# TimoStoff/event_utils

Measured on AMD Instinct MI355X. Metric: Mevents/s (voxel 5-bin 640x480), higher is better.
Workload: dtype f32

## Files before the change

### event_utils_amd/csrc/evk_part.h

```cpp
#pragma once
#include "evk_tiles.h"

namespace evk {

#define EVK_WAIT_VM0() __builtin_amdgcn_s_waitcnt(0x0F70)

struct TileGridG {
    int tw, th, pitch;
    int tiles_x, tiles_y;
    int dom_w, dom_h;
    float ix, iy;
    uint32_t mx, mp;
};
__host__ __device__ inline uint32_t magic_div(uint32_t d) { return (uint32_t)((((uint64_t)1 << 32) + d - 1) / d); }
__device__ __forceinline__ uint32_t div_magic(uint32_t x, uint32_t m) { return __umulhi(x, m); }
#define EVK_GRIDG_MAX_CELLS 1024

__device__ __forceinline__ int tile_of(int u, float inv) { return (int)(((float)u + 0.5f) * inv); }

static inline int make_grid_g(TileGridG &g, int dom_h, int dom_w, int tw, int th) {
    if (dom_h <= 0 || dom_w <= 0 || dom_h > 65535 || dom_w > 65535 || tw < 4 || th < 4 || tw > 256 || th > 256 ||
        (tw | 1) * th > EVK_GRIDG_MAX_CELLS)
        return EVK_EINVAL;
    g.tw = tw, g.th = th, g.pitch = tw | 1;
    g.dom_w = dom_w, g.dom_h = dom_h;
    g.tiles_x = (dom_w + tw - 1) / tw;
    g.tiles_y = (dom_h + th - 1) / th;
    g.ix = 1.0f / (float)tw, g.iy = 1.0f / (float)th;
    g.mx = magic_div((uint32_t)tw), g.mp = magic_div((uint32_t)(tw * th));
    return EVK_OK;
}

template <bool WRAP = true>
__device__ __forceinline__ int nearest_key_cell_int(int xi, int yi, bool finite, const TileGridG &g, uint32_t &cell) {
    if constexpr (WRAP) {
        xi += xi < 0 ? g.dom_w : 0;
        yi += yi < 0 ? g.dom_h : 0;
    }
    const bool ok = finite & ((uint32_t)xi < (uint32_t)g.dom_w) & ((uint32_t)yi < (uint32_t)g.dom_h);
    const int ux = ok ? xi : 0, uy = ok ? yi : 0;
    const int tx = tile_of(ux, g.ix), ty = tile_of(uy, g.iy);
    cell = (uint32_t)(__mul24(uy - __mul24(ty, g.th), g.pitch) + (ux - __mul24(tx, g.tw)));
    return ok ? __mul24(ty, g.tiles_x) + tx : -1;
}
__device__ __forceinline__ int nearest_key_cell(float x, float y, const TileGridG &g, uint32_t &cell) {
    return nearest_key_cell_int((int)x, (int)y, (x == x) & (y == y), g, cell);
}

struct TimeNorm {
    float t_first, dt, bm1;
};
__host__ __device__ inline TimeNorm make_time_norm(float t_first, float t_last, float bm1) {
    return TimeNorm{t_first, t_last - t_first, bm1};
}
__device__ __forceinline__ float time_norm(float t, const TimeNorm &k) { return (t - k.t_first) / k.dt * k.bm1; }

typedef uint32_t evk_u32x4 __attribute__((ext_vector_type(4)));
struct __attribute__((packed, aligned(4))) evk_quad4 {
    evk_u32x4 v;
};
template <bool NT>
__device__ __forceinline__ uint4 load_col16(const float *col, int64_t ev0, uint32_t gl) {
    const evk_quad4 *q = reinterpret_cast<const evk_quad4 *>(col + ev0) + gl;
    evk_u32x4 v;
#pragma clang diagnostic push
#pragma clang diagnostic ignored "-Waddress-of-packed-member"
    if constexpr (NT) v = __builtin_nontemporal_load(&q->v);
    else v = q->v;
#pragma clang diagnostic pop
    return make_uint4(v.x, v.y, v.z, v.w);
}
struct SrcF32 {
    static constexpr int G = 4, XYW = 8, TPW = 8;
    const float *x, *y, *t, *p;
    template <bool NT = false>
    __device__ __forceinline__ void load_xy(int64_t ev0, uint32_t gl, uint32_t *r) const {
        const uint4 a = load_col16<NT>(x, ev0, gl), b = load_col16<NT>(y, ev0, gl);
        r[0] = a.x, r[1] = a.y, r[2] = a.z, r[3] = a.w, r[4] = b.x, r[5] = b.y, r[6] = b.z, r[7] = b.w;
    }
    template <bool NT = false>
    __device__ __forceinline__ void load_tp(int64_t ev0, uint32_t gl, uint32_t *r) const {
        const uint4 a = load_col16<NT>(t, ev0, gl), b = load_col16<NT>(p, ev0, gl);
        r[0] = a.x, r[1] = a.y, r[2] = a.z, r[3] = a.w, r[4] = b.x, r[5] = b.y, r[6] = b.z, r[7] = b.w;
    }
    __device__ __forceinline__ int key_of(const uint32_t *r, int e, const TileGridG &g, uint32_t &cell) const {
        return nearest_key_cell(__uint_as_float(r[e]), __uint_as_float(r[4 + e]), g, cell);
    }
    __device__ __forceinline__ float t_of(const uint32_t *r, int e) const { return __uint_as_float(r[e]); }
    __device__ __forceinline__ float p_of(const uint32_t *r, int e) const { return __uint_as_float(r[4 + e]); }
    __device__ __forceinline__ float t1(int64_t i) const { return t[i]; }
};

template <bool T64>
struct SrcNative {
    static constexpr int G = 4, XYW = 4, TPW = T64 ? 9 : 5;
    const int16_t *x, *y;
    const void *t;
    const uint8_t *p;
    double t_offset;
    int xy_stride, p_kind;
    template <bool NT = false>
    __device__ __forceinline__ void load_xy(int64_t ev0, uint32_t gl, uint32_t *r) const {
        if (xy_stride == 2) {
            const uint4 w = reinterpret_cast<const uint4 *>(x + 2 * ev0)[gl];
            r[0] = w.x, r[1] = w.y, r[2] = w.z, r[3] = w.w;
        } else {
            const uint2 a = reinterpret_cast<const uint2 *>(x + ev0)[gl], b = reinterpret_cast<const uint2 *>(y + ev0)[gl];
            r[0] = a.x, r[1] = a.y, r[2] = b.x, r[3] = b.y;
        }
    }
    template <bool NT = false>
    __device__ __forceinline__ void load_tp(int64_t ev0, uint32_t gl, uint32_t *r) const {
        if constexpr (T64) {
            const uint4 a = reinterpret_cast<const uint4 *>(static_cast<const double *>(t) + ev0)[2 * gl];
            const uint4 b = reinterpret_cast<const uint4 *>(static_cast<const double *>(t) + ev0)[2 * gl + 1];
            r[0] = a.x, r[1] = a.y, r[2] = a.z, r[3] = a.w, r[4] = b.x, r[5] = b.y, r[6] = b.z, r[7] = b.w;
        } else {
            const uint4 a = reinterpret_cast<const uint4 *>(static_cast<const float *>(t) + ev0)[gl];
            r[0] = a.x, r[1] = a.y, r[2] = a.z, r[3] = a.w;
        }
        r[TPW - 1] = reinterpret_cast<const uint32_t *>(p + ev0)[gl];
    }
    __device__ __forceinline__ int key_of(const uint32_t *r, int e, const TileGridG &g, uint32_t &cell) const {
        const uint32_t wx = xy_stride == 2 ? r[e] << 16 : (e & 1 ? r[e >> 1] : r[e >> 1] << 16);
        const uint32_t wy = xy_stride == 2 ? r[e] : (e & 1 ? r[2 + (e >> 1)] : r[2 + (e >> 1)] << 16);
        return nearest_key_cell_int((int32_t)wx >> 16, (int32_t)wy >> 16, true, g, cell);
    }
    __device__ __forceinline__ float t_of(const uint32_t *r, int e) const {
        if constexpr (T64) {
            const double d = __hiloint2double((int)r[2 * e + 1], (int)r[2 * e]);
            return (float)(d - t_offset);
        } else {
            return (float)((double)__uint_as_float(r[e]) - t_offset);
        }
    }
    __device__ __forceinline__ float p_of(const uint32_t *r, int e) const {
        const uint32_t b = (r[TPW - 1] >> (8 * e)) & 0xffu;
        return p_kind == EVK_P_U8_PM1 ? (float)(2 * (int)b - 1) : (p_kind == EVK_P_I8 ? (float)(int8_t)b : (float)b);
    }
    __device__ __forceinline__ float t1(int64_t i) const {
        return (float)((T64 ? static_cast<const double *>(t)[i] : (double)static_cast<const float *>(t)[i]) - t_offset);
    }
};

}
```

### event_utils_amd/csrc/evk_part2.h

```cpp
#pragma once
#include <cstdio>
#include <cstring>
#include <mutex>
#include <type_traits>

#include "evk_part.h"

namespace evk {

#define V2_HDR 16
#define V2_MAX_TILES 2048
#define V2_TOTALS V2_HDR
#define V2_LIVE_PROGRESS (V2_HDR + V2_MAX_TILES)
#define V2_LIVE_STATUS (V2_LIVE_PROGRESS + 256)
#define V2_PART (V2_LIVE_STATUS + V2_MAX_TILES)
#define V2_COUNTER(T) (V2_PART + (T) + 1)
#define V2_ITEM(T) (V2_PART + 2 * (T) + 1)
#define V2_LB 10
#define EVK_VOXEL2_COUNT (1 << 20)
#define EVK_VOXEL2_COUNT2 (1 << 21)
#define V2_LOCAL_MASK ((1u << V2_LB) - 1u)
#define V2_WIDE (1u << V2_LB)
#define V2_P_MASK (~((2u << V2_LB) - 1u))
__device__ __forceinline__ void lds_barrier() { asm volatile("s_waitcnt lgkmcnt(0)\n\ts_barrier" ::: "memory"); }

template <int THREADS>
__device__ __forceinline__ uint32_t block_excl_scan(uint32_t mine, uint32_t *tmp, uint32_t &total) {
    constexpr int NW = THREADS / 64;
    const int lane = threadIdx.x & 63, wave = threadIdx.x >> 6;
    uint32_t incl = mine;
#pragma unroll
    for (int off = 1; off < 64; off <<= 1) {
        const uint32_t v = __shfl_up(incl, off, 64);
        if (lane >= off) incl += v;
    }
    if (lane == 63) tmp[wave] = incl;
    lds_barrier();
    if (wave == 0) {
        const uint32_t w = lane < NW ? tmp[lane] : 0u;
        uint32_t wi = w;
#pragma unroll
        for (int off = 1; off < NW; off <<= 1) {
            const uint32_t v = __shfl_up(wi, off, 64);
            if (lane >= off) wi += v;
        }
        if (lane < NW) tmp[32 + lane] = wi - w;
        if (lane == NW - 1) tmp[64] = wi;
    }
    lds_barrier();
    total = tmp[64];
    return tmp[32 + wave] + incl - mine;
}

__host__ __device__ static inline int64_t v2_staging_stride(int64_t cells) { return (cells + 31) & ~(int64_t)31; }

struct Part2 {
    int S;
    int per_block;
    int nsc;
    int nt_pad;
    int nblk;
};

#define V2_FMT_IMGN 1
#define V2_FMT_IMGB 12
#define V2_FMT_IMGT 13
#define V2_FMT_IMGX 14
#define V2_FMT_IMGD 15
#define V2_FMT_VOX8W 9
#define V2_DELTA_SHIFT 12
#define V2_DELTA_LIMIT (1u << 20)
#define V2_CODE_SHIFT 10
__host__ __device__ constexpr int v2_fmt_lds_bytes(int rec) { return rec == V2_FMT_IMGN ? 8 : ((rec == V2_FMT_VOX8W || rec == V2_FMT_IMGT || rec == V2_FMT_IMGX || rec == V2_FMT_IMGD) ? 12 : rec); }
template <int THREADS, int EPT, int REC, typename C, bool LIVE = false>
__global__ void __launch_bounds__(THREADS, 4) k_part_sorted(const C c, int64_t n, TileGridG g, int ntiles, Part2 q, float t_first,
                                                            float t_last, float bm1, int t_from_events,
                                                            void *__restrict__ rec_, void *__restrict__ side_,
                                                            uint32_t *__restrict__ bases,
                                                            uint32_t *__restrict__ table, uint32_t *__restrict__ index,
                                                            uint32_t cap, uint32_t part, uint32_t *oob, uint32_t *host_report,
                                                            uint32_t seq, uint32_t *live_progress = nullptr,
                                                            uint32_t live_epoch = 0) {
    static_assert(!LIVE || REC == 8, "the live consumer reads 8-byte records written through");
    static_assert(REC == 8 || REC == 4 || REC == V2_FMT_IMGN || REC == V2_FMT_IMGB || REC == V2_FMT_IMGT || REC == V2_FMT_IMGX || REC == V2_FMT_IMGD || REC == V2_FMT_VOX8W, "record format");
    constexpr bool R8 = REC == 8 || REC == V2_FMT_VOX8W;
    constexpr bool IMGBT = REC == V2_FMT_IMGB || REC == V2_FMT_IMGT || REC == V2_FMT_IMGX || REC == V2_FMT_IMGD;
    constexpr bool STAGE_W = REC == V2_FMT_VOX8W || REC == V2_FMT_IMGN || IMGBT;
    constexpr bool VOX = R8 || REC == 4;
    constexpr int LB = v2_fmt_lds_bytes(REC);
    uint2 *const rec = static_cast<uint2 *>(rec_);
    float *const pw = static_cast<float *>(side_);
    uint2 *const wide2 = static_cast<uint2 *>(side_);
    constexpr int G = C::G, NG = EPT / G;
    static_assert(EPT % G == 0, "events per thread");
    constexpr int PER_MAX = (V2_MAX_TILES + THREADS - 1) / THREADS;
    extern __shared__ __attribute__((aligned(16))) unsigned char smem[];
    uint2 *sorted = reinterpret_cast<uint2 *>(smem);
    uint32_t *hist = reinterpret_cast<uint32_t *>(smem + (size_t)THREADS * EPT * LB + 16);
    uint32_t *cur = hist + ((ntiles + 4) & ~3);
    uint32_t *tot = cur + ((ntiles + 4) & ~3);
    uint32_t *tmp = tot + ((ntiles + 4) & ~3);
    uint32_t *trow_l = tmp + 72 + 4;
    uint32_t *sorted4 = reinterpret_cast<uint32_t *>(smem);
    uint32_t *sortedp = reinterpret_cast<uint32_t *>(smem + (size_t)THREADS * EPT * (REC == V2_FMT_IMGN ? 4 : 8));
    __shared__ int is_last;
    const int tid = threadIdx.x, lane = tid & 63;
    uint32_t dropped = 0, nwide = 0;
    float tb = 0.0f;
    if constexpr (VOX) {
        if (t_from_events) t_first = c.t1(0), t_last = c.t1(n - 1);
    }
    const TimeNorm tnorm = make_time_norm(t_first, t_last, bm1);
    float ts_a = 0.0f, ts_d = 1.0f;
    if constexpr (REC == V2_FMT_IMGT) c.time_constants(n, t_from_events, ts_a, ts_d);
    constexpr bool EARLY = !IMGBT;
    uint32_t early_prev = 0;
    auto early_publish = [&]() {
        EVK_HANDOVER_ACQUIRE();
        __hip_atomic_store(index + 8, 0u, __ATOMIC_RELAXED, __HIP_MEMORY_SCOPE_AGENT);
        if (host_report) {
            const uint32_t cnt = oob ? __hip_atomic_load(oob, __ATOMIC_RELAXED, __HIP_MEMORY_SCOPE_AGENT) : 0u;
            __hip_atomic_store(reinterpret_cast<unsigned long long *>(host_report),
                               (unsigned long long)seq | ((unsigned long long)cnt << 32), __ATOMIC_RELAXED, __HIP_MEMORY_SCOPE_SYSTEM);
        }
    };

    int tl_ = tid;
    auto valid_in = [&](int sc, int k) -> int {
        const int64_t lo = (int64_t)sc * q.S;
        const int64_t hi = (lo + q.S < n) ? lo + q.S : n;
        return (int)(hi - lo) - G * (tl_ + k * THREADS);
    };
    auto row_base = [&](int sc, int k) -> int64_t {
        const int64_t lo = (int64_t)sc * q.S, hi = (lo + q.S < n) ? lo + q.S : n, r = lo + (int64_t)G * k * THREADS;
        return r < hi ? r : lo;
    };
    const int sc0 = blockIdx.x * q.per_block;
    const int sc_end = (sc0 + q.per_block < q.nsc) ? sc0 + q.per_block : q.nsc;
    uint32_t xyr[NG * C::XYW], tpr[NG * C::TPW];
    float tv[EPT];
    uint32_t kl[EPT];
    float xr[EPT], yr[EPT];
    uint32_t rare = 0;
    auto load_xy = [&](int sc) {
#pragma unroll
        for (int k = 0; k < NG; ++k) c.template load_xy<true>(row_base(sc, k), valid_in(sc, k) > 0 ? (uint32_t)tl_ : 0u, xyr + C::XYW * k);
    };
    auto load_tp = [&](int sc) {
#pragma unroll
        for (int k = 0; k < NG; ++k) c.template load_tp<true>(row_base(sc, k), valid_in(sc, k) > 0 ? (uint32_t)tl_ : 0u, tpr + C::TPW * k);
        if constexpr (REC == 4) tb = c.t1((int64_t)sc * q.S);
    };
    auto fence = [&]() {
        asm volatile("" ::: "memory");
        __builtin_amdgcn_sched_barrier(0);
    };
    for (int i = tid; i < ntiles; i += THREADS) hist[i] = 0, tot[i] = 0;
    if (tid < 8) tmp[64 + tid] = 0;
    if (sc0 < sc_end) load_xy(sc0);
    EVK_WAIT_VM0();
    lds_barrier();
    uint32_t kept_prev = 0;
    int64_t lo_prev = 0;
    int sc_prev = 0;
    auto store_run = [&](const uint4 *src, uint4 *dst, const int n16) {
        if constexpr (REC != 4) {
            typedef uint32_t u4v __attribute__((ext_vector_type(4)));
            const __amdgpu_buffer_rsrc_t rs = __builtin_amdgcn_make_buffer_rsrc(
                (void *)dst, 0, (int)__builtin_amdgcn_readfirstlane(n16 * 16), 0x00020000);
            for (int i = tid; i < n16; i += THREADS) {
                const uint4 v = src[i];
                __builtin_amdgcn_raw_buffer_store_b128(u4v{v.x, v.y, v.z, v.w}, rs, i * 16, 0,  16);
            }
        } else {
            for (int i = tid; i < n16; i += THREADS) dst[i] = src[i];
        }
    };
    auto write_out = [&]() {
        const uint4 *src = reinterpret_cast<const uint4 *>(sorted);
        if constexpr (R8 || IMGBT)
            store_run(src, reinterpret_cast<uint4 *>(rec + lo_prev), (int)((kept_prev + 1) >> 1));
        else
            store_run(src, reinterpret_cast<uint4 *>(reinterpret_cast<uint32_t *>(rec_) + lo_prev), (int)((kept_prev + 3) >> 2));
        if constexpr (LIVE)
            store_run(reinterpret_cast<const uint4 *>(trow_l), reinterpret_cast<uint4 *>(table + (int64_t)sc_prev * q.nt_pad), q.nt_pad >> 2);
        if constexpr (STAGE_W) {
            if (tmp[65])
                store_run(reinterpret_cast<const uint4 *>(sortedp),
                          reinterpret_cast<uint4 *>(static_cast<uint32_t *>(side_) + lo_prev), (int)((kept_prev + 3) >> 2));
        }
    };
    for (int sc = sc0; sc < sc_end; ++sc) {
        asm volatile("" : "+v"(tl_));
        const int64_t lo = (int64_t)sc * q.S;
        if (sc > sc0) write_out();
#pragma unroll
        for (int k = 0; k < NG; ++k) {
            const int nv = valid_in(sc, k);
#pragma unroll
            for (int e = 0; e < G; ++e) {
                uint32_t cell = 0;
                int key;
                if constexpr (IMGBT) key = c.key_rel(xyr + C::XYW * k, e, g, xr[G * k + e], yr[G * k + e]);
                else key = c.key_of(xyr + C::XYW * k, e, g, cell);
                kl[G * k + e] = ((key >= 0) & (e < nv)) ? (((uint32_t)key << V2_LB) | cell) : 0xFFFFFFFFu;
                if constexpr (VOX) dropped += ((key < 0) & (e < nv)) ? 1u : 0u;
                else dropped += ((key == -1) & (e < nv)) ? 1u : 0u;
                if constexpr (IMGBT) rare |= ((key == -3) & (e < nv)) ? (1u << (G * k + e)) : 0u;
                asm volatile("" : "+v"(dropped));
                __builtin_amdgcn_sched_barrier(0);
            }
        }
#pragma unroll
        for (int s2 = 0; s2 < EPT; ++s2) asm volatile("" : "+v"(kl[s2])::"memory");
        load_tp(sc);
#pragma unroll
        for (int s2 = 0; s2 < EPT; ++s2)
            if (kl[s2] != 0xFFFFFFFFu)
                __hip_atomic_fetch_add(&hist[kl[s2] >> V2_LB], 1u, __ATOMIC_RELAXED, __HIP_MEMORY_SCOPE_WORKGROUP);
        if constexpr (EARLY) {
            if (sc == sc_end - 1 && dropped) __hip_atomic_fetch_add(&tmp[69], dropped, __ATOMIC_RELAXED, __HIP_MEMORY_SCOPE_WORKGROUP);
        }
        lds_barrier();
        if constexpr (EARLY) {
            if (sc == sc_end - 1 && tid == 0 && oob && tmp[69])
                __hip_atomic_fetch_add(oob, tmp[69], __ATOMIC_RELAXED, __HIP_MEMORY_SCOPE_AGENT);
        }
        uint32_t kept = 0;
        {
            uint32_t *trow = table + (int64_t)sc * q.nt_pad;
            constexpr int NWV = THREADS / 64;
            const int wave = tid >> 6;
            for (int base = 0; base < ntiles; base += THREADS) {
                const int i = base + tid;
                const uint32_t cnt = i < ntiles ? hist[i] : 0u;
                uint32_t incl = cnt;
#pragma unroll
                for (int off = 1; off < 64; off <<= 1) {
                    const uint32_t v = __shfl_up(incl, off, 64);
                    if (lane >= off) incl += v;
                }
                if (lane == 63) tmp[wave] = incl;
                lds_barrier();
                const uint32_t wt = lane < NWV ? tmp[lane] : 0u;
                uint32_t wi = wt;
#pragma unroll
                for (int off = 1; off < NWV; off <<= 1) {
                    const uint32_t v = __shfl_up(wi, off, 64);
                    if (lane >= off) wi += v;
                }
                const uint32_t carry = kept + __shfl(wi - wt, wave, 64);
                if (i < ntiles) {
                    const uint32_t start = carry + incl - cnt;
                    cur[i] = start;
                    hist[i] = 0;
                    tot[i] += cnt;
                    if constexpr (LIVE) trow_l[i] = start | (cnt << 16);
                    else trow[i] = start | (cnt << 16);
                }
                kept += __shfl(wi, NWV - 1, 64);
                if (base + THREADS < ntiles) lds_barrier();
            }
            if (REC == 4 && tid == 0) tmp[67] = 0;
            if (STAGE_W && tid == 0) tmp[65] = 0;
        }
        lds_barrier();
        if constexpr (VOX) {
#pragma unroll
            for (int s2 = 0; s2 < EPT; ++s2) {
                tv[s2] = time_norm(c.t_of(tpr + C::TPW * (s2 / G), s2 % G), tnorm);
                __builtin_amdgcn_sched_barrier(0);
            }
        }
        EVK_WAIT_VM0();
        fence();
        if constexpr (EARLY) {
            if (sc == sc_end - 1 && tid == 0) {
                EVK_HANDOVER_RELEASE();
                early_prev = __hip_atomic_fetch_add(index + 8, 1u, __ATOMIC_RELAXED, __HIP_MEMORY_SCOPE_AGENT);
            }
        }
        if (sc + 1 < sc_end) load_xy(sc + 1);
        fence();
        uint32_t pos_[EPT];
#pragma unroll
        for (int s2 = 0; s2 < EPT; ++s2) {
            pos_[s2] = 0;
            if (kl[s2] != 0xFFFFFFFFu) pos_[s2] = atomicAdd(&cur[kl[s2] >> V2_LB], 1u);
        }
        auto slot_of = [&](int s2) -> uint32_t { return pos_[s2]; };
        if constexpr (REC == V2_FMT_VOX8W) {
            bool any_wide = false;
#pragma unroll
            for (int s2 = 0; s2 < EPT; ++s2) {
                if (kl[s2] != 0xFFFFFFFFu) {
                    const uint32_t pos = slot_of(s2);
                    const uint32_t pbits = __float_as_uint(c.p_of(tpr + C::TPW * (s2 / G), s2 % G));
                    const bool wide = ((pbits & ~V2_P_MASK) != 0u) | ((pbits & 0x7F800000u) == 0x7F800000u);
                    nwide += ((((pbits & 0x7FFFFFFFu) == 0x3F800000u) | (pbits == 0u)) ? 0u : 0x10000u) + (wide ? 1u : 0u);
                    sorted[pos] = make_uint2(__float_as_uint(tv[s2]), (wide ? V2_WIDE : (pbits & V2_P_MASK)) | (kl[s2] & V2_LOCAL_MASK));
                    sortedp[pos] = pbits;
                    any_wide |= wide;
                }
            }
            if (any_wide) tmp[65] = 1u;
        } else if constexpr (REC == 8) {
            uint32_t wide_mask = 0;
#pragma unroll
            for (int s2 = 0; s2 < EPT; ++s2) {
                if (kl[s2] != 0xFFFFFFFFu) {
                    const uint32_t pos = slot_of(s2);
                    const uint32_t pbits = __float_as_uint(c.p_of(tpr + C::TPW * (s2 / G), s2 % G));
                    const bool wide = ((pbits & ~V2_P_MASK) != 0u) | ((pbits & 0x7F800000u) == 0x7F800000u);
                    nwide += (((pbits & 0x7FFFFFFFu) == 0x3F800000u) | (pbits == 0u)) ? 0u : 0x10000u;
                    sorted[pos] = make_uint2(__float_as_uint(tv[s2]), (wide ? V2_WIDE : (pbits & V2_P_MASK)) | (kl[s2] & V2_LOCAL_MASK));
                    if (wide) wide_mask |= 1u << s2, kl[s2] = pos;
                }
            }
            if (__any(wide_mask != 0u)) {
#pragma unroll
                for (int s2 = 0; s2 < EPT; ++s2)
                    if (wide_mask >> s2 & 1u) pw[lo + kl[s2]] = c.p_of(tpr + C::TPW * (s2 / G), s2 % G), ++nwide;
            }
        } else if constexpr (REC == V2_FMT_IMGN) {
            bool any_wide = false;
#pragma unroll
            for (int s2 = 0; s2 < EPT; ++s2) {
                if (kl[s2] != 0xFFFFFFFFu) {
                    const uint32_t pos = slot_of(s2);
                    bool wide, unit;
                    const uint32_t pay = c.payload(tpr + C::TPW * (s2 / G), s2 % G, wide, unit);
                    nwide += (unit ? 0u : 0x10000u) + (wide ? 1u : 0u);
                    sorted4[pos] = (wide ? V2_WIDE : (pay & V2_P_MASK)) | (kl[s2] & V2_LOCAL_MASK);
                    sortedp[pos] = c.w_bits(tpr + C::TPW * (s2 / G), s2 % G);
                    any_wide |= wide;
                }
            }
            if (any_wide) tmp[65] = 1u;
        } else if constexpr (REC == V2_FMT_IMGB || REC == V2_FMT_IMGX) {
            bool any_b = false;
#pragma unroll
            for (int s2 = 0; s2 < EPT; ++s2) {
                if (kl[s2] != 0xFFFFFFFFu) {
                    const uint32_t pos = slot_of(s2);
                    const uint32_t wb = c.w_bits(tpr + C::TPW * (s2 / G), s2 % G);
                    const uint32_t code = (wb & 0x7FFFFFFFu) == 0x3F800000u ? wb >> 31 : 3u - (uint32_t)(wb == 0u);
                    nwide += code == 3u ? 0x10001u : 0u;
                    sorted[pos] = make_uint2((__float_as_uint(xr[s2]) & 0x7FFFFFFFu) | (code << 31),
                                             (__float_as_uint(yr[s2]) & 0x7FFFFFFFu) | ((code >> 1) << 31));
                    sortedp[pos] = wb;
                    any_b |= code == 3u;
                }
            }
            if (any_b) tmp[65] = 1u;
            if (__any(rare != 0u)) {
#pragma unroll
                for (int s2 = 0; s2 < EPT; ++s2)
                    if (rare >> s2 & 1u) {
                        if constexpr (REC == V2_FMT_IMGX)
                            dropped += c.rare_at(row_base(sc, s2 / G) + (int64_t)G * tl_ + (s2 % G)) ? 0u : 1u;
                        else
                            dropped += c.rare(xr[s2], yr[s2], __uint_as_float(c.w_bits(tpr + C::TPW * (s2 / G), s2 % G))) ? 0u : 1u;
                    }
            }
            rare = 0;
        } else if constexpr (REC == V2_FMT_IMGD) {
            bool any_d = false;
#pragma unroll
            for (int s2 = 0; s2 < EPT; ++s2) {
                if (kl[s2] != 0xFFFFFFFFu) {
                    const uint32_t pos = slot_of(s2);
                    sorted[pos] = make_uint2(__float_as_uint(xr[s2]), __float_as_uint(yr[s2]));
                    sortedp[pos] = (uint32_t)(row_base(sc, s2 / G) + (int64_t)G * tl_ + (s2 % G));
                    any_d = true;
                }
            }
            if (any_d) tmp[65] = 1u;
            if (__any(rare != 0u)) {
#pragma unroll
                for (int s2 = 0; s2 < EPT; ++s2)
                    if (rare >> s2 & 1u) dropped += c.rare_at(row_base(sc, s2 / G) + (int64_t)G * tl_ + (s2 % G)) ? 0u : 1u;
            }
            rare = 0;
        } else if constexpr (REC == V2_FMT_IMGT) {
            bool any_t = false;
#pragma unroll
            for (int s2 = 0; s2 < EPT; ++s2) {
                if (kl[s2] != 0xFFFFFFFFu) {
                    const uint32_t pos = slot_of(s2);
                    const uint32_t cls = c.cls(tpr + C::TPW * (s2 / G), s2 % G);
                    sorted[pos] = make_uint2((__float_as_uint(xr[s2]) & 0x7FFFFFFFu) | ((cls & 1u) << 31),
                                             (__float_as_uint(yr[s2]) & 0x7FFFFFFFu) | ((cls >> 1) << 31));
                    sortedp[pos] = c.nts_bits(tpr + C::TPW * (s2 / G), s2 % G, ts_a, ts_d);
                    any_t = true;
                }
            }
            if (any_t) tmp[65] = 1u;
            if (__any(rare != 0u)) {
#pragma unroll
                for (int s2 = 0; s2 < EPT; ++s2)
                    if (rare >> s2 & 1u) dropped += c.rare_ts(xr[s2], yr[s2], tpr + C::TPW * (s2 / G), s2 % G, ts_a, ts_d) ? 0u : 1u;
            }
            rare = 0;
        } else {
            const uint32_t bbits = __float_as_uint(time_norm(tb, tnorm));
            if (tid == 0) bases[sc] = bbits;
#pragma unroll
            for (int s2 = 0; s2 < EPT; ++s2) {
                const uint32_t tbits = __float_as_uint(tv[s2]), pb = __float_as_uint(c.p_of(tpr + C::TPW * (s2 / G), s2 % G));
                const uint32_t d = tbits - bbits;
                const uint32_t code = (pb & 0x7FFFFFFFu) == 0x3F800000u ? pb >> 31 : 3u - (uint32_t)(pb == 0u);
                const bool live = kl[s2] != 0xFFFFFFFFu;
                nwide += (live & (code == 3u)) ? 0x10000u : 0u;
                const bool esc = live & ((code == 3u) | (d >= V2_DELTA_LIMIT));
                uint32_t word = (d << V2_DELTA_SHIFT) | (code << V2_CODE_SHIFT) | (kl[s2] & V2_LOCAL_MASK);
                if (__any(esc)) {
                    if (esc) {
                        const uint32_t e = atomicAdd(&tmp[67], 1u);
                        wide2[lo + e] = make_uint2(tbits, pb);
                        word = (e << V2_DELTA_SHIFT) | (3u << V2_CODE_SHIFT) | (kl[s2] & V2_LOCAL_MASK);
                        ++nwide;
                    }
                }
                if (live) sorted4[slot_of(s2)] = word;
            }
        }
        lds_barrier();
        if constexpr (EARLY) {
            if (sc == sc_end - 1 && tid == 0 && early_prev == gridDim.x - 1) early_publish();
        }
        if constexpr (LIVE) {
            if (sc > sc0 && tid == 0)
                __hip_atomic_store(live_progress + blockIdx.x, (live_epoch << 8) | (uint32_t)(sc - sc0), __ATOMIC_RELAXED,
                                   __HIP_MEMORY_SCOPE_AGENT);
        }
        EVK_WAIT_VM0();
        kept_prev = kept, lo_prev = lo, sc_prev = sc;
    }
    uint32_t *gidx = index;
    if constexpr (EARLY) {
        if (sc0 >= sc_end && tid == 0) {
            early_prev = __hip_atomic_fetch_add(index + 8, 1u, __ATOMIC_RELAXED, __HIP_MEMORY_SCOPE_AGENT);
            if (early_prev == gridDim.x - 1) early_publish();
        }
    } else {
        if (dropped && oob) atomicAdd(oob, dropped);
    }
    for (int i = tid; i < ntiles; i += THREADS)
        if (tot[i]) __hip_atomic_fetch_add(gidx + V2_TOTALS + i, tot[i], __ATOMIC_RELAXED, __HIP_MEMORY_SCOPE_AGENT);
    {
        uint32_t nw = nwide & 0xFFFFu, nu = nwide >> 16;
#pragma unroll
        for (int off = 32; off >= 1; off >>= 1) nw += __shfl_xor(nw, off, 64), nu += __shfl_xor(nu, off, 64);
        if (lane == 0) {
            if (nw) __hip_atomic_fetch_add(&tmp[66], nw, __ATOMIC_RELAXED, __HIP_MEMORY_SCOPE_WORKGROUP);
            if (nu) __hip_atomic_fetch_add(&tmp[68], nu, __ATOMIC_RELAXED, __HIP_MEMORY_SCOPE_WORKGROUP);
        }
    }
    if (sc0 < sc_end) write_out();
    lds_barrier();
    if (tid == 0) {
        const uint32_t nw = tmp[66], nu = tmp[68];
        if (nw) __hip_atomic_fetch_add(gidx + 3, nw, __ATOMIC_RELAXED, __HIP_MEMORY_SCOPE_AGENT);
        if (nu) __hip_atomic_fetch_add(gidx + 5, nu, __ATOMIC_RELAXED, __HIP_MEMORY_SCOPE_AGENT);
    }
    if constexpr (VOX) {
        if (blockIdx.x == 0 && tid == 0 && n > 0) {
            __hip_atomic_store(gidx + 0, __float_as_uint(c.t1(0)), __ATOMIC_RELAXED, __HIP_MEMORY_SCOPE_AGENT);
            __hip_atomic_store(gidx + 1, __float_as_uint(c.t1(n - 1)), __ATOMIC_RELAXED, __HIP_MEMORY_SCOPE_AGENT);
        }
    }
    EVK_HANDOVER_DRAIN();
    if constexpr (LIVE) {
        if (sc0 < sc_end && tid == 0)
            __hip_atomic_store(live_progress + blockIdx.x, (live_epoch << 8) | (uint32_t)(sc_end - sc0), __ATOMIC_RELAXED,
                               __HIP_MEMORY_SCOPE_AGENT);
    }
    if (tid == 0) {
        const uint32_t prev = __hip_atomic_fetch_add(gidx + 2, 1u, __ATOMIC_RELAXED, __HIP_MEMORY_SCOPE_AGENT);
        is_last = (prev == gridDim.x - 1);
    }
    __syncthreads();
    if (!is_last) return;
    EVK_HANDOVER_ACQUIRE();
    const int per = (ntiles + THREADS - 1) / THREADS;
    const int i0 = tid * per, i1 = (i0 + per < ntiles) ? i0 + per : ntiles;
    uint32_t *part_start = index + V2_PART, *counters = index + V2_COUNTER(ntiles), *item_tile = index + V2_ITEM(ntiles);
    uint32_t tt[PER_MAX];
    uint32_t np = 0;
    uint32_t now5 = 0, prev6 = 0, cnt_oob = 0, now3 = 0, prev0 = 0;
    if (tid == 0) {
        now5 = __hip_atomic_load(gidx + 5, __ATOMIC_RELAXED, __HIP_MEMORY_SCOPE_AGENT);
        prev6 = __hip_atomic_load(gidx + 6, __ATOMIC_RELAXED, __HIP_MEMORY_SCOPE_AGENT);
        if constexpr (!VOX) {
            now3 = __hip_atomic_load(gidx + 3, __ATOMIC_RELAXED, __HIP_MEMORY_SCOPE_AGENT);
            prev0 = __hip_atomic_load(gidx + 0, __ATOMIC_RELAXED, __HIP_MEMORY_SCOPE_AGENT);
        }
        if (!EARLY && host_report && oob) cnt_oob = __hip_atomic_load(oob, __ATOMIC_RELAXED, __HIP_MEMORY_SCOPE_AGENT);
    }
#pragma unroll
    for (int k = 0; k < PER_MAX; ++k) {
        const int i = i0 + k;
        tt[k] = 0;
        if (k < per && i < i1) {
            tt[k] = __hip_atomic_load(gidx + V2_TOTALS + i, __ATOMIC_RELAXED, __HIP_MEMORY_SCOPE_AGENT);
            __hip_atomic_store(gidx + V2_TOTALS + i, 0u, __ATOMIC_RELAXED, __HIP_MEMORY_SCOPE_AGENT);
            np += tt[k] > cap ? (tt[k] + part - 1) / part : 1u;
        }
    }
    uint32_t total_parts;
    uint32_t prun = block_excl_scan<THREADS>(np, tmp, total_parts);
#pragma unroll
    for (int k = 0; k < PER_MAX; ++k) {
        const int i = i0 + k;
        if (k < per && i < i1) {
            const uint32_t parts = tt[k] > cap ? (tt[k] + part - 1) / part : 1u;
            part_start[i] = prun;
            counters[i] = 0;
            for (uint32_t jj = 0; jj < parts; ++jj) item_tile[prun + jj] = (uint32_t)i;
            prun += parts;
        }
    }
    if (tid == 0) {
        part_start[ntiles] = total_parts;
        __hip_atomic_store(gidx + 2, 0u, __ATOMIC_RELAXED, __HIP_MEMORY_SCOPE_AGENT);
        __hip_atomic_store(gidx + 7, now5 != prev6 ? 1u : 0u, __ATOMIC_RELAXED, __HIP_MEMORY_SCOPE_AGENT);
        __hip_atomic_store(gidx + 6, now5, __ATOMIC_RELAXED, __HIP_MEMORY_SCOPE_AGENT);
        if constexpr (!VOX) {
            __hip_atomic_store(gidx + 1, now3 != prev0 ? 1u : 0u, __ATOMIC_RELAXED, __HIP_MEMORY_SCOPE_AGENT);
            __hip_atomic_store(gidx + 0, now3, __ATOMIC_RELAXED, __HIP_MEMORY_SCOPE_AGENT);
        }
        if (!EARLY && host_report) {
            const uint32_t cnt = cnt_oob;
            __hip_atomic_store(reinterpret_cast<unsigned long long *>(host_report),
                               (unsigned long long)seq | ((unsigned long long)cnt << 32), __ATOMIC_RELAXED, __HIP_MEMORY_SCOPE_SYSTEM);
        }
    }
}

struct V2Config {
    int threads, ept;
};
#define V2_GEOMETRIES(X) X(1024, 8) X(1024, 12)
static const V2Config &v2_config(bool share = false, int ntiles = 0) {
    static const V2Config small{1024, 8}, large{1024, 12};
    return (share || ntiles <= 680) ? small : large;
}
#define V2_MIN_SUBCHUNK 8192
#define V2_LDS_LIMIT (160 * 1024 - 512)
static size_t v2_part_lds(int threads, int ept, int rec, int ntiles, bool live = false) {
    return (size_t)threads * ept * v2_fmt_lds_bytes(rec) + 16 + 3 * (size_t)((ntiles + 4) & ~3) * 4 + 72 * 4 + 16 +
           (live ? (size_t)((ntiles + 15) & ~15) * 4 + 16 : 0);
}

static Part2 v2_geometry(int64_t n, int ntiles, bool share = false) {
    const V2Config &c = v2_config(share, ntiles);
    const int64_t smax = (int64_t)c.threads * c.ept;
    int64_t nblk = (n + V2_MIN_SUBCHUNK - 1) / V2_MIN_SUBCHUNK;
    const int64_t maxblk = (int64_t)EVK_NUM_CU * (1024 / c.threads);
    if (nblk > maxblk) nblk = maxblk;
    if (nblk < 1) nblk = 1;
    int64_t per_block = (n + nblk * smax - 1) / (nblk * smax);
    if (per_block < 1) per_block = 1;
    int64_t S = (n + nblk * per_block - 1) / (nblk * per_block);
    S = (S + 3) & ~(int64_t)3;
    if (S < 4) S = 4;
    Part2 q;
    q.S = (int)S, q.per_block = (int)per_block, q.nblk = (int)nblk;
    q.nsc = (int)((n + S - 1) / S);
    if (q.nsc < 1) q.nsc = 1;
    q.nt_pad = (ntiles + 15) & ~15;
    return q;
}
static inline int64_t al256(int64_t b) { return (b + 255) & ~(int64_t)255; }

#define V2_SPLIT_AT 2.5
#define V2_SPLIT_PART 1.6
static int64_t v2_mean(int64_t n, int ntiles) { return n / (ntiles > 0 ? ntiles : 1); }
static int64_t v2_cap(int64_t n, int ntiles) {
    const int64_t c = (int64_t)(V2_SPLIT_AT * (double)v2_mean(n, ntiles));
    return c > 16384 ? c : 16384;
}
static int64_t v2_part(int64_t n, int ntiles) {
    const int64_t c = (int64_t)(V2_SPLIT_PART * (double)v2_mean(n, ntiles));
    return c > 8192 ? c : 8192;
}
static int v2_max_items(int64_t n, int ntiles) { return ntiles + (int)(n / v2_part(n, ntiles)) + 1; }

static int v2_rec_bytes(int64_t n, int flags) {
    if (flags & EVK_VOXEL2_REC4) return 4;
    if (flags & EVK_VOXEL2_REC8) return 8;
    return n * 16 > ((int64_t)256 << 20) ? 4 : 8;
}
struct V2Layout {
    int64_t table, bases, rec, pw, staging, total;
};
static V2Layout v2_layout(int ntiles, int64_t n, int planes, int tw, int th, bool share = false) {
    const Part2 q = v2_geometry(n, ntiles, share);
    const int64_t slots = (int64_t)q.nsc * q.S;
    V2Layout L;
    L.table = 0;
    L.bases = al256((int64_t)q.nsc * q.nt_pad * 4);
    L.rec = L.bases + al256((int64_t)q.nsc * 4);
    L.pw = L.rec + al256(slots * 8);
    L.staging = L.pw + al256(slots * 8);
    L.total = L.staging + al256((int64_t)v2_max_items(n, ntiles) * v2_staging_stride((int64_t)planes * tw * th) * 8);
    return L;
}

template <int THREADS, int EPT, int REC, typename C, bool LIVE = false>
static void launch_part(const C &c, int64_t n, const TileGridG &g, int ntiles, const Part2 &q, float t_first, float t_last,
                        float bm1, int t_from_events, void *rec, void *pw, uint32_t *bases, uint32_t *table, uint32_t *index,
                        uint32_t *oob, uint32_t *host_report, uint32_t seq, hipStream_t s, uint32_t *live_progress = nullptr,
                        uint32_t live_epoch = 0) {
    const size_t lds = v2_part_lds(THREADS, EPT, REC, ntiles, LIVE);
    static std::once_flag once[64];
    int dev = 0;
    (void)hipGetDevice(&dev);
    std::call_once(once[dev & 63], [] {
        (void)hipFuncSetAttribute((const void *)k_part_sorted<THREADS, EPT, REC, C, LIVE>, hipFuncAttributeMaxDynamicSharedMemorySize,
                                  160 * 1024 - 256);
    });
    k_part_sorted<THREADS, EPT, REC, C, LIVE><<<q.nblk, THREADS, lds, s>>>(c, n, g, ntiles, q, t_first, t_last, bm1, t_from_events,
                                                                          rec, pw, bases, table, index, (uint32_t)v2_cap(n, ntiles), (uint32_t)v2_part(n, ntiles), oob,
                                                                          host_report, seq, live_progress, live_epoch);
}

}
```

Measured before the change: 140,600.

## Deepen load pipeline: issue t/p loads early and prefetch next xy during binning

For small EPT with 8, 4 or VOX8W record formats, the partition kernel now issues the t/p column loads at the top of each supertile and prefetches the next supertile's x/y right after key computation. Partial vmcnt waits (a new EVK_WAIT_VM(N) macro) replace full drains, so outstanding loads overlap the histogram, scan and scatter phases. Per-source constants give the number of load instructions per column group so the waits count correctly. This keeps more memory traffic in flight and holds more live registers, and it relies on the vmcnt arithmetic being exact or the data read will be stale.

```diff
diff --git a/event_utils_amd/csrc/evk_part.h b/event_utils_amd/csrc/evk_part.h
--- a/event_utils_amd/csrc/evk_part.h
+++ b/event_utils_amd/csrc/evk_part.h
@@ -4,6 +4,7 @@
 namespace evk {
 
 #define EVK_WAIT_VM0() __builtin_amdgcn_s_waitcnt(0x0F70)
+#define EVK_WAIT_VM(N) __builtin_amdgcn_s_waitcnt(0x0F70 | ((N) & 15) | (((N) >> 4) << 14))
 
 struct TileGridG {
     int tw, th, pitch;
@@ -72,6 +73,7 @@
 }
 struct SrcF32 {
     static constexpr int G = 4, XYW = 8, TPW = 8;
+    static constexpr int XYL = 2, TPL = 2;
     const float *x, *y, *t, *p;
     template <bool NT = false>
     __device__ __forceinline__ void load_xy(int64_t ev0, uint32_t gl, uint32_t *r) const {
@@ -94,6 +96,7 @@
 template <bool T64>
 struct SrcNative {
     static constexpr int G = 4, XYW = 4, TPW = T64 ? 9 : 5;
+    static constexpr int XYL = 1, TPL = T64 ? 3 : 2;
     const int16_t *x, *y;
     const void *t;
     const uint8_t *p;
diff --git a/event_utils_amd/csrc/evk_part2.h b/event_utils_amd/csrc/evk_part2.h
--- a/event_utils_amd/csrc/evk_part2.h
+++ b/event_utils_amd/csrc/evk_part2.h
@@ -72,6 +72,7 @@
 #define V2_DELTA_LIMIT (1u << 20)
 #define V2_CODE_SHIFT 10
 __host__ __device__ constexpr int v2_fmt_lds_bytes(int rec) { return rec == V2_FMT_IMGN ? 8 : ((rec == V2_FMT_VOX8W || rec == V2_FMT_IMGT || rec == V2_FMT_IMGX || rec == V2_FMT_IMGD) ? 12 : rec); }
+__host__ __device__ constexpr int v2_pipe_depth(int ept, int rec) { return (ept <= 8 && (rec == 8 || rec == 4 || rec == V2_FMT_VOX8W)) ? 2 : 1; }
 template <int THREADS, int EPT, int REC, typename C, bool LIVE = false>
 __global__ void __launch_bounds__(THREADS, 4) k_part_sorted(const C c, int64_t n, TileGridG g, int ntiles, Part2 q, float t_first,
                                                             float t_last, float bm1, int t_from_events,
@@ -88,6 +89,7 @@
     constexpr bool STAGE_W = REC == V2_FMT_VOX8W || REC == V2_FMT_IMGN || IMGBT;
     constexpr bool VOX = R8 || REC == 4;
     constexpr int LB = v2_fmt_lds_bytes(REC);
+    constexpr bool DEEP = v2_pipe_depth(EPT, REC) == 2;
     uint2 *const rec = static_cast<uint2 *>(rec_);
     float *const pw = static_cast<float *>(side_);
     uint2 *const wide2 = static_cast<uint2 *>(side_);
@@ -142,9 +144,9 @@
     uint32_t kl[EPT];
     float xr[EPT], yr[EPT];
     uint32_t rare = 0;
-    auto load_xy = [&](int sc) {
-#pragma unroll
-        for (int k = 0; k < NG; ++k) c.template load_xy<true>(row_base(sc, k), valid_in(sc, k) > 0 ? (uint32_t)tl_ : 0u, xyr + C::XYW * k);
+    auto load_xy = [&](int sc, bool real = true) {
+#pragma unroll
+        for (int k = 0; k < NG; ++k) c.template load_xy<true>(row_base(sc, k), (valid_in(sc, k) > 0 && real) ? (uint32_t)tl_ : 0u, xyr + C::XYW * k);
     };
     auto load_tp = [&](int sc) {
 #pragma unroll
@@ -158,7 +160,7 @@
     for (int i = tid; i < ntiles; i += THREADS) hist[i] = 0, tot[i] = 0;
     if (tid < 8) tmp[64 + tid] = 0;
     if (sc0 < sc_end) load_xy(sc0);
-    EVK_WAIT_VM0();
+    if constexpr (!DEEP) EVK_WAIT_VM0();
     lds_barrier();
     uint32_t kept_prev = 0;
     int64_t lo_prev = 0;
@@ -193,6 +195,11 @@
     for (int sc = sc0; sc < sc_end; ++sc) {
         asm volatile("" : "+v"(tl_));
         const int64_t lo = (int64_t)sc * q.S;
+        if constexpr (DEEP) {
+            load_tp(sc);
+            EVK_WAIT_VM(NG * C::TPL);
+            fence();
+        }
         if (sc > sc0) write_out();
 #pragma unroll
         for (int k = 0; k < NG; ++k) {
@@ -213,7 +220,11 @@
         }
 #pragma unroll
         for (int s2 = 0; s2 < EPT; ++s2) asm volatile("" : "+v"(kl[s2])::"memory");
-        load_tp(sc);
+        if constexpr (DEEP) {
+            load_xy(sc + 1 < sc_end ? sc + 1 : sc, sc + 1 < sc_end);
+        } else {
+            load_tp(sc);
+        }
 #pragma unroll
         for (int s2 = 0; s2 < EPT; ++s2)
             if (kl[s2] != 0xFFFFFFFFu)
@@ -265,6 +276,11 @@
             if (STAGE_W && tid == 0) tmp[65] = 0;
         }
         lds_barrier();
+        if constexpr (DEEP) {
+            if constexpr (LIVE) EVK_WAIT_VM0();
+            else EVK_WAIT_VM(NG * C::XYL);
+            fence();
+        }
         if constexpr (VOX) {
 #pragma unroll
             for (int s2 = 0; s2 < EPT; ++s2) {
@@ -272,16 +288,19 @@
                 __builtin_amdgcn_sched_barrier(0);
             }
         }
-        EVK_WAIT_VM0();
+        if constexpr (!DEEP) EVK_WAIT_VM0();
         fence();
         if constexpr (EARLY) {
             if (sc == sc_end - 1 && tid == 0) {
+                if constexpr (DEEP) EVK_WAIT_VM0();
                 EVK_HANDOVER_RELEASE();
                 early_prev = __hip_atomic_fetch_add(index + 8, 1u, __ATOMIC_RELAXED, __HIP_MEMORY_SCOPE_AGENT);
             }
         }
-        if (sc + 1 < sc_end) load_xy(sc + 1);
-        fence();
+        if constexpr (!DEEP) {
+            if (sc + 1 < sc_end) load_xy(sc + 1);
+            fence();
+        }
         uint32_t pos_[EPT];
 #pragma unroll
         for (int s2 = 0; s2 < EPT; ++s2) {
@@ -434,7 +453,8 @@
                 __hip_atomic_store(live_progress + blockIdx.x, (live_epoch << 8) | (uint32_t)(sc - sc0), __ATOMIC_RELAXED,
                                    __HIP_MEMORY_SCOPE_AGENT);
         }
-        EVK_WAIT_VM0();
+        if constexpr (!DEEP)
+            EVK_WAIT_VM0();
         kept_prev = kept, lo_prev = lo, sc_prev = sc;
     }
     uint32_t *gidx = index;
```

New measurement: 129,000. 0.918x the previous value.
